# nubot-nudt/MDGAT-matcher

Measured on AMD Instinct MI355X. Metric: keypoint-pairs/sec, higher is better.
Workload: dtype f32 (products as 3 split-f16 MFMAs, fp32 accumulate)

## Files before the change

mdgat_matcher_amd/csrc/layer.hip:

```cpp
#include <utility>
#include <cstdlib>
#include "common.hpp"
#include "layer_image.hpp"
#include "mma_chain.hpp"
namespace {

constexpr int SLOT_CHUNKS = 17;
constexpr int SLOT_BYTES = SLOT_CHUNKS * 1024;
constexpr int SLOT_HALVES = SLOT_BYTES / 2;
constexpr int NSLOT = 5, LOOKAHEAD = 3;
constexpr int WPTS = 16;
constexpr int TROW = 132;
constexpr int TILE_FLOATS = WPTS * TROW;
constexpr int QKROW = 72;
constexpr int VROW = 24;

typedef f16x8 __attribute__((may_alias)) f16x8_a;
typedef f16x4 __attribute__((may_alias)) f16x4_a;
typedef f32x4 __attribute__((may_alias)) f32x4_a;

template <int NW>
__device__ __forceinline__ void stage_dma_slice(const _Float16* g, unsigned lds_addr, int wave, int lane, int i) {
    const int c = min(wave + NW * i, SLOT_CHUNKS - 1);
    const char* src = reinterpret_cast<const char*>(g) + c * 1024;
    asm volatile("s_mov_b32 m0, %0\n\ts_nop 0\n\tglobal_load_lds_dwordx4 %1, %2"
                 :: "s"(lds_addr + c * 1024), "v"(lane * 16), "s"(src) : "memory");
}
template <int NW> constexpr int dma_slices() { return (SLOT_CHUNKS + NW - 1) / NW; }
template <int NW>
__device__ __forceinline__ void stage_dma(const _Float16* g, unsigned lds_addr, int wave, int lane) {
#pragma unroll
    for (int i = 0; i < dma_slices<NW>(); ++i) stage_dma_slice<NW>(g, lds_addr, wave, lane, i);
}
template <typename F, int... U>
__device__ __forceinline__ void for_each_unit(F&& f, std::integer_sequence<int, U...>) { (f(U), ...); }
template <int N, typename F>
__device__ __forceinline__ void for_units(F&& f) { for_each_unit(f, std::make_integer_sequence<int, N>{}); }

template <int YOUNGER>
__device__ __forceinline__ void stage_wait() {
    asm volatile("s_waitcnt vmcnt(%0)" :: "n"(YOUNGER) : "memory");
    __syncthreads();
}
template <int NW>
__device__ __forceinline__ void end_of_pair(int h1, int nstage) {
    if (h1 + 3 < nstage) stage_wait<dma_slices<NW>()>();
    else stage_wait<0>();
}

struct UnitAcc { f32x4 pm, px, qm, qx; };

template <int NK32, bool SWAP, int ROWH, typename Inter>
__device__ __forceinline__ void unit_mma16(const _Float16* buf, int l15, int g, const f16x8* xh, const f16x8* xl,
                                           UnitAcc& acc, Inter&& inter) {
    constexpr int K = NK32 * 32, AHEAD = 2;
    const _Float16* wp = buf + l15 * ROWH + 8 * g;
    const _Float16* wq = wp + 16 * ROWH;
    acc.pm = f32x4{0.f, 0.f, 0.f, 0.f}; acc.px = acc.pm; acc.qm = acc.pm; acc.qx = acc.pm;
    f16x8 ph[NK32], pl[NK32], qh[NK32], ql[NK32];
#pragma unroll
    for (int ks = 0; ks < AHEAD; ++ks) {
        ph[ks] = *reinterpret_cast<const f16x8*>(wp + 32 * ks);
        pl[ks] = *reinterpret_cast<const f16x8*>(wp + K + 32 * ks);
        qh[ks] = *reinterpret_cast<const f16x8*>(wq + 32 * ks);
        ql[ks] = *reinterpret_cast<const f16x8*>(wq + K + 32 * ks);
    }
    auto mm = [&](const f16x8& w, const f16x8& x, const f32x4& c) __attribute__((always_inline)) {
        return SWAP ? __builtin_amdgcn_mfma_f32_16x16x32_f16(w, x, c, 0, 0, 0)
                    : __builtin_amdgcn_mfma_f32_16x16x32_f16(x, w, c, 0, 0, 0);
    };
#pragma unroll
    for (int ks = 0; ks < NK32; ++ks) {
        if (ks + AHEAD < NK32) {
            ph[ks + AHEAD] = *reinterpret_cast<const f16x8*>(wp + 32 * (ks + AHEAD));
            pl[ks + AHEAD] = *reinterpret_cast<const f16x8*>(wp + K + 32 * (ks + AHEAD));
            qh[ks + AHEAD] = *reinterpret_cast<const f16x8*>(wq + 32 * (ks + AHEAD));
            ql[ks + AHEAD] = *reinterpret_cast<const f16x8*>(wq + K + 32 * (ks + AHEAD));
        }
        __builtin_amdgcn_sched_barrier(0);
        acc.px = mm(ph[ks], xl[ks], acc.px); inter(6 * ks); __builtin_amdgcn_sched_barrier(0);
        acc.qx = mm(qh[ks], xl[ks], acc.qx); inter(6 * ks + 1); __builtin_amdgcn_sched_barrier(0);
        acc.pm = mm(ph[ks], xh[ks], acc.pm); inter(6 * ks + 2); __builtin_amdgcn_sched_barrier(0);
        acc.qm = mm(qh[ks], xh[ks], acc.qm); inter(6 * ks + 3); __builtin_amdgcn_sched_barrier(0);
        acc.px = mm(pl[ks], xh[ks], acc.px); inter(6 * ks + 4); __builtin_amdgcn_sched_barrier(0);
        acc.qx = mm(ql[ks], xh[ks], acc.qx); inter(6 * ks + 5); __builtin_amdgcn_sched_barrier(0);
    }
}

template <int NK32, int ROWH, typename Inter>
__device__ __forceinline__ void block_mma16(const _Float16* buf, int l15, int g, const f16x8* xh, const f16x8* xl,
                                            f32x4& m, f32x4& x, Inter&& inter) {
    constexpr int K = NK32 * 32, AHEAD = 3;
    const _Float16* wp = buf + l15 * ROWH + 8 * g;
    m = f32x4{0.f, 0.f, 0.f, 0.f}; x = m;
    f16x8 ph[NK32], pl[NK32];
#pragma unroll
    for (int ks = 0; ks < AHEAD; ++ks) {
        ph[ks] = *reinterpret_cast<const f16x8*>(wp + 32 * ks);
        pl[ks] = *reinterpret_cast<const f16x8*>(wp + K + 32 * ks);
    }
#pragma unroll
    for (int ks = 0; ks < NK32; ++ks) {
        if (ks + AHEAD < NK32) {
            ph[ks + AHEAD] = *reinterpret_cast<const f16x8*>(wp + 32 * (ks + AHEAD));
            pl[ks + AHEAD] = *reinterpret_cast<const f16x8*>(wp + K + 32 * (ks + AHEAD));
        }
        __builtin_amdgcn_sched_barrier(0);
        x = __builtin_amdgcn_mfma_f32_16x16x32_f16(ph[ks], xl[ks], x, 0, 0, 0); inter(3 * ks); __builtin_amdgcn_sched_barrier(0);
        m = __builtin_amdgcn_mfma_f32_16x16x32_f16(ph[ks], xh[ks], m, 0, 0, 0); inter(3 * ks + 1); __builtin_amdgcn_sched_barrier(0);
        x = __builtin_amdgcn_mfma_f32_16x16x32_f16(pl[ks], xh[ks], x, 0, 0, 0); inter(3 * ks + 2); __builtin_amdgcn_sched_barrier(0);
    }
}

template <int DO_MLP, int MODE3, int VW, int NW>
__global__ __launch_bounds__(64 * NW) void layer_kernel(LayerArgs a) {
    constexpr int NWAVE = NW, DMA_SLICES = dma_slices<NW>();
    static_assert(!VW || NW == 8, "the V^T gather buffers are laid out for 128-keypoint workgroups");
    extern __shared__ __attribute__((aligned(16))) _Float16 smem[];
    const int tid = threadIdx.x;
    const int lane = tid & 63;
    const int wave = __builtin_amdgcn_readfirstlane(tid >> 6);
    const int l15 = lane & 15, g = lane >> 4;
    auto bufp = [&](int i) __attribute__((always_inline)) { return smem + (i % NSLOT) * SLOT_HALVES; };
    const unsigned lds0 = (unsigned)(size_t)(__attribute__((address_space(3))) _Float16*)smem;
    auto ldsb = [&](int i) __attribute__((always_inline)) { return lds0 + (unsigned)(i % NSLOT) * SLOT_BYTES; };
    float* bias1 = reinterpret_cast<float*>(smem + NSLOT * SLOT_HALVES);
    float* bias2 = bias1 + 256;
    float* bias3 = bias2 + 128;
    float* tile = bias3 + 384 + wave * TILE_FLOATS;
    _Float16* tile16 = reinterpret_cast<_Float16*>(tile);
    constexpr int NT = 64 * NWAVE, TILE_PTS = WPTS * NWAVE;
    const int wave_pt0 = blockIdx.x * TILE_PTS + wave * WPTS;
    constexpr int NB3 = MODE3 == 1 ? 12 : 4;

    constexpr int NSTAGE = (DO_MLP ? 24 : 0) + NB3;
    auto stage_src = [&](int h) __attribute__((always_inline)) -> const _Float16* {
        if (DO_MLP && h < 16) return a.w1s + (size_t)h * 16 * ROWH256;
        if (DO_MLP && h < 24) return a.w2s + (size_t)(h - 16) * 16 * ROWH256;
        return a.w3s + (size_t)(h - (DO_MLP ? 24 : 0)) * 32 * ROWH128;
    };
    auto copy_ahead = [&](int h, int i) __attribute__((always_inline)) {
        if (h + LOOKAHEAD < NSTAGE) stage_dma_slice<NW>(stage_src(h + LOOKAHEAD), ldsb(h + LOOKAHEAD), wave, lane, i);
    };
    if (DO_MLP) {
#pragma unroll
        for (int i = tid; i < 256; i += NT) bias1[i] = a.b1[i];
#pragma unroll
        for (int i = tid; i < 128; i += NT) bias2[i] = a.b2[i];
    }
#pragma unroll
    for (int i = tid; i < NB3 * 32; i += NT) bias3[i] = a.b3[i];

    const int l31 = lane & 31, hi = lane >> 5;
    auto rows_load = [&](const float* src, f32x4 (&t)[8]) __attribute__((always_inline)) {
#pragma unroll
        for (int i = 0; i < 8; ++i) {
            const int gp = min(wave_pt0 + 2 * i + hi, a.R - 1);
            t[i] = *reinterpret_cast<const f32x4*>(src + (size_t)gp * 128 + l31 * 4);
        }
    };
    auto rows_guard = [&](const f32x4 (&t)[8], unsigned acc) __attribute__((always_inline)) -> unsigned {
#pragma unroll
        for (int i = 0; i < 8; ++i)
#pragma unroll
            for (int c = 0; c < 4; c += 2)
                acc = max(acc, max(__builtin_bit_cast(unsigned, t[i][c]) & 0x7fffffffu, __builtin_bit_cast(unsigned, t[i][c + 1]) & 0x7fffffffu));
        return acc;
    };
    auto guard_report = [&](unsigned acc) __attribute__((always_inline)) {
        if (a.guard && acc >= __builtin_bit_cast(unsigned, MDGAT_F16_GUARD))
            __hip_atomic_store(a.guard, 1u, __ATOMIC_RELAXED, __HIP_MEMORY_SCOPE_SYSTEM);
    };
    auto rows_to_tile = [&](const f32x4 (&t)[8]) __attribute__((always_inline)) {
#pragma unroll
        for (int i = 0; i < 8; ++i) *reinterpret_cast<f32x4_a*>(tile + (2 * i + hi) * TROW + l31 * 4) = t[i];
    };
    auto tile_to_rows = [&](float* dst) __attribute__((always_inline)) {
#pragma unroll
        for (int i = 0; i < 8; ++i) {
            const int p = 2 * i + hi;
            const f32x4 t = *reinterpret_cast<const f32x4_a*>(tile + p * TROW + l31 * 4);
            const int gp = min(wave_pt0 + p, a.R - 1);
            *reinterpret_cast<f32x4*>(dst + (size_t)gp * 128 + l31 * 4) = t;
        }
    };
    auto tile_fragment = [&](int ks, f16x8& h, f16x8& l) __attribute__((always_inline)) {
        float v[8];
        load8(tile + l15 * TROW + 32 * ks + 8 * g, v);
        split8s(v, h, l);
    };

    UnitAcc acc[2];
    float o[8];
    f16x8 xnh[4], xnl[4];

    float pbias[8], pv[8], phf[8];
    float pbias_v[2] = {0.f, 0.f};
    f16x8 sth, stl;
    f32x4 pback[2];
    constexpr int E_STEPS = 16;

    auto combine = [&](const UnitAcc& c, int half) __attribute__((always_inline)) {
#pragma unroll
        for (int r = 0; r < 4; ++r)
            o[4 * half + r] = half == 0 ? fmaf(c.px[r], MDGAT_SPLIT_INV, c.pm[r]) : fmaf(c.qx[r], MDGAT_SPLIT_INV, c.qm[r]);
    };
    auto load_bias8 = [&](const float* b) __attribute__((always_inline)) { load8(b + 8 * g, pbias); };
    auto split_step = [&](int s_, f16x8& h, f16x8& l, bool SCALED = true) __attribute__((always_inline)) {
        typedef unsigned u32x4 __attribute__((ext_vector_type(4)));
        if (s_ == 0) {
#pragma unroll
            for (int j = 0; j < 8; ++j) h[j] = (_Float16)pv[j];
        } else if (s_ == 1) {
            const u32x4 hp = __builtin_bit_cast(u32x4, h);
#pragma unroll
            for (int j = 0; j < 4; ++j) {
                asm("v_fma_mix_f32 %0, %1, 1.0, -%2 op_sel:[0,0,0] op_sel_hi:[0,0,1]" : "=v"(pv[2 * j]) : "v"(pv[2 * j]), "v"(hp[j]));
                asm("v_fma_mix_f32 %0, %1, 1.0, -%2 op_sel:[0,0,1] op_sel_hi:[0,0,1]" : "=v"(pv[2 * j + 1]) : "v"(pv[2 * j + 1]), "v"(hp[j]));
            }
        } else if (s_ == 2) {
            if (SCALED) {
#pragma unroll
                for (int j = 0; j < 8; ++j) pv[j] *= MDGAT_SPLIT_SCALE;
            }
        } else if (s_ == 3) {
#pragma unroll
            for (int j = 0; j < 8; ++j) l[j] = (_Float16)pv[j];
        }
    };

    constexpr int VSH_OFF = 16 * QKROW, VSHROW = 136, VSH_BUF = 8 * VSHROW;
    _Float16* tiles16 = reinterpret_cast<_Float16*>(bias3 + 384);
    auto vsh = [&](int b, int row, int col) __attribute__((always_inline)) {
        return tiles16 + (row >> 3) * (2 * TILE_FLOATS) + VSH_OFF + b * VSH_BUF + (row & 7) * VSHROW + col;
    };
    auto vstore = [&](int qb, int u) __attribute__((always_inline)) {
        const int p = u >> 1, rl = 4 * p + g;
        if ((u & 1) == 0) pback[p] = *reinterpret_cast<const f32x4_a*>(tile16 + VSH_OFF + (qb & 1) * VSH_BUF + rl * VSHROW + l15 * 8);
        else {
            const int P = a.N + a.M;
            const int pt0 = blockIdx.x * (WPTS * NWAVE);
            const int bb = pt0 / P, pp = pt0 - bb * P;
            const int col0 = pp < a.N ? pp : a.Npad + pp - a.N;
            _Float16* base = a.vt16 + (((size_t)bb * 4 + (qb & 3)) * 64 + 8 * wave + rl) * a.PP + col0;
            *reinterpret_cast<f32x4*>(base + l15 * 8) = pback[p];
        }
    };

    auto e3 = [&](int qb, const UnitAcc& c, int u) __attribute__((always_inline)) {
        if (u == 1 || u == 2) { combine(c, u - 1); return; }
        if (MODE3 == 1 && qb < 8) {
            if (u == 0) load_bias8(bias3 + qb * 32);
            else if (u == 3) {
#pragma unroll
                for (int j = 0; j < 8; ++j) pv[j] = o[j] + pbias[j];
            } else if (u == 4) {
                if (qb < 4) {
#pragma unroll
                    for (int j = 0; j < 8; ++j) pv[j] *= MDGAT_LOG2E * 0.17677669529663687f;
                }
            } else if (u <= 9) split_step(u - 5, sth, stl, false);
            else if (u == 10) {
                *reinterpret_cast<f16x8_a*>(tile16 + l15 * QKROW + 8 * g) = sth;
                *reinterpret_cast<f16x8_a*>(tile16 + l15 * QKROW + 32 + 8 * g) = stl;
            } else if (u == 11) {
#pragma unroll
                for (int p = 0; p < 2; ++p)
                    pback[p] = *reinterpret_cast<const f32x4_a*>(tile16 + (8 * p + (lane >> 3)) * QKROW + (lane & 7) * 8);
            } else if (u <= 13) {
                const int p = u - 12;
                _Float16* dst = (qb < 4 ? a.q16 : a.k16) + (size_t)(qb & 3) * 64;
                const int row = 8 * p + (lane >> 3), cc = lane & 7;
                const int gp = min(wave_pt0 + row, a.R - 1);
                *reinterpret_cast<f32x4*>(dst + (size_t)gp * 256 + cc * 8) = pback[p];
            }
        } else if (MODE3 == 1) {
            const int head = qb & 3;
            const int P = a.N + a.M;
            if (VW) {
                if (u == 0) { pbias_v[0] = bias3[qb * 32 + l15]; pbias_v[1] = bias3[qb * 32 + 16 + l15]; }
                else if (u == 3) {
#pragma unroll
                    for (int j = 0; j < 8; ++j) pv[j] = o[j] + pbias_v[j >> 2];
                } else if (u >= 5 && u <= 9) split_step(u - 5, sth, stl, false);
                else if (u == 10) {
                    _Float16* c0 = vsh(qb & 1, l15, 16 * wave + 4 * g);
                    *reinterpret_cast<f16x4_a*>(c0) = f16x4{sth[0], sth[1], sth[2], sth[3]};
                    *reinterpret_cast<f16x4_a*>(c0 + 2 * 2 * TILE_FLOATS) = f16x4{sth[4], sth[5], sth[6], sth[7]};
                    *reinterpret_cast<f16x4_a*>(c0 + 4 * 2 * TILE_FLOATS) = f16x4{stl[0], stl[1], stl[2], stl[3]};
                    *reinterpret_cast<f16x4_a*>(c0 + 6 * 2 * TILE_FLOATS) = f16x4{stl[4], stl[5], stl[6], stl[7]};
                }
            } else if (((a.N | a.M) & 15) == 0) {
                if (wave_pt0 < a.R) {
                    if (u == 0) { pbias_v[0] = bias3[qb * 32 + l15]; pbias_v[1] = bias3[qb * 32 + 16 + l15]; }
                    else if (u == 3) {
#pragma unroll
                        for (int j = 0; j < 8; ++j) pv[j] = o[j] + pbias_v[j >> 2];
                    } else if (u >= 5 && u <= 9) split_step(u - 5, sth, stl, false);
                    else if (u == 10) {
                        *reinterpret_cast<f16x4_a*>(tile16 + l15 * VROW + 4 * g) = f16x4{sth[0], sth[1], sth[2], sth[3]};
                        *reinterpret_cast<f16x4_a*>(tile16 + (16 + l15) * VROW + 4 * g) = f16x4{sth[4], sth[5], sth[6], sth[7]};
                        *reinterpret_cast<f16x4_a*>(tile16 + (32 + l15) * VROW + 4 * g) = f16x4{stl[0], stl[1], stl[2], stl[3]};
                        *reinterpret_cast<f16x4_a*>(tile16 + (48 + l15) * VROW + 4 * g) = f16x4{stl[4], stl[5], stl[6], stl[7]};
                    } else if (u == 11) {
#pragma unroll
                        for (int p = 0; p < 2; ++p)
                            pback[p] = *reinterpret_cast<const f32x4_a*>(tile16 + lane * VROW + p * 8);
                    } else if (u == 12 || u == 13) {
                        const int p = u - 12;
                        const int bb = wave_pt0 / P, pp = wave_pt0 - bb * P;
                        const int col0 = pp < a.N ? pp : a.Npad + pp - a.N;
                        _Float16* base = a.vt16 + ((size_t)bb * 4 + head) * 64 * a.PP + col0;
                        *reinterpret_cast<f32x4*>(base + (size_t)lane * a.PP + p * 8) = pback[p];
                    }
                }
            } else if (u == 11) {
                const bool fast = ((a.N | a.M) & 3) == 0;
                const int p0 = wave_pt0 + 4 * g;
#pragma unroll
                for (int blk = 0; blk < 2; ++blk) {
                    if (p0 >= a.R) continue;
                    const int dim = 16 * blk + l15;
                    const float bias = bias3[qb * 32 + dim];
                    _Float16 h[4], l[4];
#pragma unroll
                    for (int j = 0; j < 4; ++j) mdgat_split_unscaled(o[4 * blk + j] + bias, h[j], l[j]);
                    if (fast) {
                        const int bb = p0 / P, pp = p0 - bb * P;
                        _Float16* row_h = a.vt16 + (((size_t)bb * 4 + head) * 2 * 32 + dim) * a.PP;
                        const int col = pp < a.N ? pp : a.Npad + pp - a.N;
                        *reinterpret_cast<f16x4*>(row_h + col) = f16x4{h[0], h[1], h[2], h[3]};
                        *reinterpret_cast<f16x4*>(row_h + (size_t)32 * a.PP + col) = f16x4{l[0], l[1], l[2], l[3]};
                    } else {
#pragma unroll
                        for (int j = 0; j < 4; ++j) {
                            const int pj = p0 + j;
                            if (pj >= a.R) break;
                            const int bj = pj / P, qj = pj - bj * P;
                            const int col = qj < a.N ? qj : a.Npad + qj - a.N;
                            _Float16* rh = a.vt16 + (((size_t)bj * 4 + head) * 2 * 32 + dim) * a.PP;
                            rh[col] = h[j];
                            rh[(size_t)32 * a.PP + col] = l[j];
                        }
                    }
                }
            }
        } else {
            if (u == 0) load_bias8(bias3 + qb * 32);
            else if (u == 3) {
#pragma unroll
                for (int j = 0; j < 8; ++j) pv[j] = o[j] + pbias[j];
            } else if (u == 4) store8(tile + l15 * TROW + qb * 32 + 8 * g, pv);
        }
    };

    if (DO_MLP) {
        f16x8 ah[8], al[8];
        {
            f32x4 tm[8], tx[8];
            rows_load(a.msg, tm);
            rows_load(a.x, tx);
            for_units<LOOKAHEAD>([&](int h) __attribute__((always_inline)) { stage_dma<NW>(stage_src(h), ldsb(h), wave, lane); });
            rows_to_tile(tm);
            const unsigned gm = rows_guard(tm, 0u);
            for_units<4>([&](int ks) __attribute__((always_inline)) { tile_fragment(ks, ah[4 + ks], al[4 + ks]); });
            rows_to_tile(tx);
            guard_report(rows_guard(tx, gm));
        }
        for_units<4>([&](int ks) __attribute__((always_inline)) { tile_fragment(ks, ah[ks], al[ks]); });
        stage_wait<DMA_SLICES>();

        f16x8 hh[8], hl[8];
        auto e1 = [&](int rb, const UnitAcc& c, int u) __attribute__((always_inline)) {
            if (u == 0) load_bias8(bias1 + rb * 32);
            else if (u <= 2) combine(c, u - 1);
            else if (u == 3) {
#pragma unroll
                for (int j = 0; j < 8; ++j) pv[j] = o[j] + pbias[j];
            } else if (u == 4) {
#pragma unroll
                for (int j = 0; j < 8; ++j) pv[j] = fmaxf(pv[j], 0.f);
            } else if (u <= 9) split_step(u - 5, hh[rb], hl[rb]);
        };
        for_units<8>([&](int rb) __attribute__((always_inline)) {
            auto inter = [&](int h, int base) __attribute__((always_inline)) {
                return [&, h, base](int slot) __attribute__((always_inline)) {
                    if (slot % 4 == 1 && slot / 4 < DMA_SLICES) copy_ahead(h, slot / 4);
                    if (slot % 2 == 0 && rb > 0) e1(rb - 1, acc[(rb - 1) & 1], (base + slot) / 2);
                };
            };
            block_mma16<8, ROWH256>(bufp(2 * rb), l15, g, ah, al, acc[rb & 1].pm, acc[rb & 1].px, inter(2 * rb, 0));
            block_mma16<8, ROWH256>(bufp(2 * rb + 1), l15, g, ah, al, acc[rb & 1].qm, acc[rb & 1].qx, inter(2 * rb + 1, 24));
            end_of_pair<NW>(2 * rb + 1, NSTAGE);
        });

        auto e2 = [&](int ob, const UnitAcc& c, int u) __attribute__((always_inline)) {
            if (u == 0) {
                load_bias8(bias2 + ob * 32);
                load8(tile + l15 * TROW + ob * 32 + 8 * g, phf);
            } else if (u <= 2) combine(c, u - 1);
            else if (u == 3) {
#pragma unroll
                for (int j = 0; j < 8; ++j) pv[j] = o[j] + pbias[j];
            } else if (u == 4) {
#pragma unroll
                for (int j = 0; j < 8; ++j) pv[j] += phf[j];
            } else if (u == 5) store8(tile + l15 * TROW + ob * 32 + 8 * g, pv);
            else if (u <= 10) split_step(u - 6, xnh[ob], xnl[ob]);
        };
        for_units<4>([&](int ob) __attribute__((always_inline)) {
            constexpr int H0 = 16;
            auto inter = [&](int h, int base) __attribute__((always_inline)) {
                return [&, h, base](int slot) __attribute__((always_inline)) {
                    if (slot % 4 == 1 && slot / 4 < DMA_SLICES) copy_ahead(h, slot / 4);
                    if (slot % 2 != 0) return;
                    if (ob == 0) e1(7, acc[1], (base + slot) / 2);
                    else e2(ob - 1, acc[(ob - 1) & 1], (base + slot) / 2);
                };
            };
            block_mma16<8, ROWH256>(bufp(H0 + 2 * ob), l15, g, hh, hl, acc[ob & 1].pm, acc[ob & 1].px, inter(H0 + 2 * ob, 0));
            block_mma16<8, ROWH256>(bufp(H0 + 2 * ob + 1), l15, g, hh, hl, acc[ob & 1].qm, acc[ob & 1].qx, inter(H0 + 2 * ob + 1, 24));
            end_of_pair<NW>(H0 + 2 * ob + 1, NSTAGE);
        });
        for_units<E_STEPS>([&](int u) __attribute__((always_inline)) { e2(3, acc[1], u); });
        tile_to_rows(a.x);
    } else {
        {
            f32x4 tx[8];
            rows_load(a.x, tx);
            for_units<LOOKAHEAD>([&](int h) __attribute__((always_inline)) { stage_dma<NW>(stage_src(h), ldsb(h), wave, lane); });
            rows_to_tile(tx);
            guard_report(rows_guard(tx, 0u));
        }
        for_units<4>([&](int ks) __attribute__((always_inline)) { tile_fragment(ks, xnh[ks], xnl[ks]); });
        stage_wait<DMA_SLICES>();
    }

    for_units<NB3>([&](int q) __attribute__((always_inline)) {
        constexpr int H0 = DO_MLP ? 24 : 0;
        const _Float16* cur = bufp(H0 + q);
        auto inter = [&](int slot) __attribute__((always_inline)) {
            if (slot % 4 == 1 && slot / 4 < DMA_SLICES) copy_ahead(H0 + q, slot / 4);
            if (q > 0) e3(q - 1, acc[(q - 1) & 1], slot);
            if (VW && q >= 10 && slot >= 18 && slot < 22) vstore(q - 2, slot - 18);
        };
        if (MODE3 == 1 && q >= 8) unit_mma16<4, false, ROWH128>(cur, l15, g, xnh, xnl, acc[q & 1], inter);
        else unit_mma16<4, true, ROWH128>(cur, l15, g, xnh, xnl, acc[q & 1], inter);
        if ((q & 1) && q + 1 < NB3) end_of_pair<NW>(H0 + q, NSTAGE);
        else if (VW && q >= 10) __syncthreads();
    });
    if (VW) for_units<4>([&](int u) __attribute__((always_inline)) { vstore(NB3 - 2, u); });
    for_units<E_STEPS>([&](int u) __attribute__((always_inline)) { e3(NB3 - 1, acc[(NB3 - 1) & 1], u); });
    if (VW) {
        __syncthreads();
        for_units<4>([&](int u) __attribute__((always_inline)) { vstore(NB3 - 1, u); });
    }
    if (MODE3 != 1) tile_to_rows(a.mdesc);
}

__global__ __launch_bounds__(256) void split_rows_kernel(const float* w, _Float16* out, int rows, int K, int rowh, int nperm) {
    const size_t total = (size_t)rows * K;
    for (size_t i = (size_t)blockIdx.x * 256 + threadIdx.x; i < total; i += (size_t)gridDim.x * 256) {
        const int r = (int)(i / K), c = (int)(i - (size_t)r * K);
        int src = r;
        if (r < nperm) {
            const int j = r & 15, q = (r >> 4) & 1;
            src = (r & ~31) + 8 * (j >> 2) + 4 * q + (j & 3);
        }
        _Float16 h, l;
        mdgat_split(w[(size_t)src * K + c], h, l);
        out[(size_t)r * rowh + c] = h;
        out[(size_t)r * rowh + K + c] = l;
    }
}

template <int DO_MLP, int MODE3, int VW, int NW>
int launch_layer_t(const LayerArgs& a, hipStream_t s) {
    constexpr int NWAVE = NW;
    const size_t lds = (size_t)NSLOT * SLOT_BYTES + (768 + NWAVE * TILE_FLOATS) * sizeof(float);
    static std::atomic<unsigned long long> optin;
    if (int rc = mdgat_lds_optin(reinterpret_cast<const void*>(layer_kernel<DO_MLP, MODE3, VW, NW>), lds, optin, "layer LDS attribute")) return rc;
    constexpr int TILE_PTS = WPTS * NWAVE;
    hipLaunchKernelGGL((layer_kernel<DO_MLP, MODE3, VW, NW>), dim3((a.R + TILE_PTS - 1) / TILE_PTS), dim3(64 * NWAVE), lds, s, a);
    return mdgat_check_hip(hipGetLastError(), "layer launch");
}

}

int launch_split_rows(const float* w, _Float16* out, int rows, int K, int rowh, int nperm, hipStream_t s) {
    const size_t total = (size_t)rows * K;
    const int blocks = (int)((total + 255) / 256 < 1024 ? (total + 255) / 256 : 1024);
    hipLaunchKernelGGL(split_rows_kernel, dim3(blocks), dim3(256), 0, s, w, out, rows, K, rowh, nperm);
    return mdgat_check_hip(hipGetLastError(), "split_rows launch");
}

static std::atomic<int> g_split_tiles{[] { const char* e = getenv("MDGAT_LAYER_SPLIT_TILES"); return e ? atoi(e) : MDGAT_LAYER_SPLIT_TILES_DEFAULT; }()};
extern "C" int mdgat_set_layer_split_tiles(int tiles) { return g_split_tiles.exchange(tiles < 0 ? MDGAT_LAYER_SPLIT_TILES_DEFAULT : tiles); }

int launch_layer(const LayerLaunch& p, hipStream_t s) {
    if (p.R <= 0) return MDGAT_OK;
    LayerArgs a{};
    a.x = p.x; a.msg = p.msg;
    a.w1s = p.mlp.w1s; a.b1 = p.mlp.b1; a.w2s = p.mlp.w2s; a.b2 = p.mlp.b2; a.w3s = p.proj.w3s; a.b3 = p.proj.b3;
    a.w1f = p.mlp.w1f; a.w2f = p.mlp.w2f; a.w3f = p.proj.w3f;
    a.q16 = p.out.q16; a.k16 = p.out.k16; a.vt16 = p.out.vt16; a.mdesc = p.mdesc;
    a.R = p.R; a.N = p.N; a.M = p.M; a.Npad = p.out.Npad; a.PP = p.out.PP; a.guard = p.guard;
    if ((p.R + 127) / 128 <= g_split_tiles.load(std::memory_order_relaxed)) return launch_layer_split(a, p.do_mlp, p.proj.mode3, s);
    if ((p.R + 127) / 128 <= MDGAT_LAYER_TILE64_TILES) {
        if (p.do_mlp) return p.proj.mode3 != 1 ? launch_layer_t<1, 2, 0, 4>(a, s) : launch_layer_t<1, 1, 0, 4>(a, s);
        return p.proj.mode3 != 1 ? launch_layer_t<0, 2, 0, 4>(a, s) : launch_layer_t<0, 1, 0, 4>(a, s);
    }
    const bool vw = p.proj.mode3 == 1 && ((p.N | p.M) & 127) == 0;
    if (p.do_mlp) return p.proj.mode3 != 1 ? launch_layer_t<1, 2, 0, 8>(a, s) : vw ? launch_layer_t<1, 1, 1, 8>(a, s) : launch_layer_t<1, 1, 0, 8>(a, s);
    return p.proj.mode3 != 1 ? launch_layer_t<0, 2, 0, 8>(a, s) : vw ? launch_layer_t<0, 1, 1, 8>(a, s) : launch_layer_t<0, 1, 0, 8>(a, s);
}
```

Before: 21310.

## Replace per-wave LDS transpose tiles with cross-lane permutes and direct register stores

Removes the per-wave fp32 LDS tile used to transpose rows into MFMA fragments and back. Input rows are loaded in a layout where ds_bpermute and permlane16_swap move data into fragment ownership, and outputs (mdesc, x residual, q/k/v f16) are stored straight from registers. The residual is kept in registers, and the V^T gather buffer is placed in a free weight ring slot. This cuts LDS footprint (a static_assert sizes it so an attention workgroup can share the CU) and LDS round trips, at the cost of more permute instructions, held registers, and narrower global stores.

```diff
diff --git a/mdgat_matcher_amd/csrc/layer.hip b/mdgat_matcher_amd/csrc/layer.hip
--- a/mdgat_matcher_amd/csrc/layer.hip
+++ b/mdgat_matcher_amd/csrc/layer.hip
@@ -10,14 +10,11 @@
 constexpr int SLOT_HALVES = SLOT_BYTES / 2;
 constexpr int NSLOT = 5, LOOKAHEAD = 3;
 constexpr int WPTS = 16;
-constexpr int TROW = 132;
-constexpr int TILE_FLOATS = WPTS * TROW;
-constexpr int QKROW = 72;
-constexpr int VROW = 24;
-
-typedef f16x8 __attribute__((may_alias)) f16x8_a;
+constexpr int LAYER_LDS_BYTES = NSLOT * SLOT_BYTES + 768 * (int)sizeof(float);
+static_assert(LAYER_LDS_BYTES <= 163840 - 67584, "the layer kernel shares its CU's LDS with one attention_stream_kernel workgroup");
 typedef f16x4 __attribute__((may_alias)) f16x4_a;
 typedef f32x4 __attribute__((may_alias)) f32x4_a;
+typedef unsigned u32x4 __attribute__((ext_vector_type(4)));
 
 template <int NW>
 __device__ __forceinline__ void stage_dma_slice(const _Float16* g, unsigned lds_addr, int wave, int lane, int i) {
@@ -115,7 +112,7 @@
 template <int DO_MLP, int MODE3, int VW, int NW>
 __global__ __launch_bounds__(64 * NW) void layer_kernel(LayerArgs a) {
     constexpr int NWAVE = NW, DMA_SLICES = dma_slices<NW>();
-    static_assert(!VW || NW == 8, "the V^T gather buffers are laid out for 128-keypoint workgroups");
+    static_assert(!VW || (NW == 8 && MODE3 == 1), "the V^T gather buffers are laid out for 128-keypoint workgroups");
     extern __shared__ __attribute__((aligned(16))) _Float16 smem[];
     const int tid = threadIdx.x;
     const int lane = tid & 63;
@@ -127,8 +124,6 @@
     float* bias1 = reinterpret_cast<float*>(smem + NSLOT * SLOT_HALVES);
     float* bias2 = bias1 + 256;
     float* bias3 = bias2 + 128;
-    float* tile = bias3 + 384 + wave * TILE_FLOATS;
-    _Float16* tile16 = reinterpret_cast<_Float16*>(tile);
     constexpr int NT = 64 * NWAVE, TILE_PTS = WPTS * NWAVE;
     const int wave_pt0 = blockIdx.x * TILE_PTS + wave * WPTS;
     constexpr int NB3 = MODE3 == 1 ? 12 : 4;
@@ -151,13 +146,28 @@
 #pragma unroll
     for (int i = tid; i < NB3 * 32; i += NT) bias3[i] = a.b3[i];
 
-    const int l31 = lane & 31, hi = lane >> 5;
+    const int gp = min(wave_pt0 + l15, a.R - 1);
     auto rows_load = [&](const float* src, f32x4 (&t)[8]) __attribute__((always_inline)) {
+        const float* row = src + (size_t)min(wave_pt0 + (lane >> 2), a.R - 1) * 128 + 8 * (lane & 3);
+#pragma unroll
+        for (int i = 0; i < 8; ++i) t[i] = *reinterpret_cast<const f32x4*>(row + 32 * (i >> 1) + 4 * (i & 1));
+    };
+    auto rows_own = [&](f32x4 (&t)[8]) __attribute__((always_inline)) {
+        const int from = 4 * (4 * l15 + g);
 #pragma unroll
         for (int i = 0; i < 8; ++i) {
-            const int gp = min(wave_pt0 + 2 * i + hi, a.R - 1);
-            t[i] = *reinterpret_cast<const f32x4*>(src + (size_t)gp * 128 + l31 * 4);
-        }
+            const u32x4 w = __builtin_bit_cast(u32x4, t[i]);
+            u32x4 r;
+#pragma unroll
+            for (int d = 0; d < 4; ++d) r[d] = (unsigned)__builtin_amdgcn_ds_bpermute(from, (int)w[d]);
+            t[i] = __builtin_bit_cast(f32x4, r);
+        }
+    };
+    auto late = [&](int v) __attribute__((always_inline)) { asm volatile("" : "+v"(v)); return v; };
+    auto unit_store = [&](float* dst, int unit, const float (&v)[8]) __attribute__((always_inline)) {
+        float* row = dst + (size_t)late(gp) * 128 + 32 * unit + 8 * g;
+        *reinterpret_cast<f32x4*>(row) = f32x4{v[0], v[1], v[2], v[3]};
+        *reinterpret_cast<f32x4*>(row + 4) = f32x4{v[4], v[5], v[6], v[7]};
     };
     auto rows_guard = [&](const f32x4 (&t)[8], unsigned acc) __attribute__((always_inline)) -> unsigned {
 #pragma unroll
@@ -171,22 +181,8 @@
         if (a.guard && acc >= __builtin_bit_cast(unsigned, MDGAT_F16_GUARD))
             __hip_atomic_store(a.guard, 1u, __ATOMIC_RELAXED, __HIP_MEMORY_SCOPE_SYSTEM);
     };
-    auto rows_to_tile = [&](const f32x4 (&t)[8]) __attribute__((always_inline)) {
-#pragma unroll
-        for (int i = 0; i < 8; ++i) *reinterpret_cast<f32x4_a*>(tile + (2 * i + hi) * TROW + l31 * 4) = t[i];
-    };
-    auto tile_to_rows = [&](float* dst) __attribute__((always_inline)) {
-#pragma unroll
-        for (int i = 0; i < 8; ++i) {
-            const int p = 2 * i + hi;
-            const f32x4 t = *reinterpret_cast<const f32x4_a*>(tile + p * TROW + l31 * 4);
-            const int gp = min(wave_pt0 + p, a.R - 1);
-            *reinterpret_cast<f32x4*>(dst + (size_t)gp * 128 + l31 * 4) = t;
-        }
-    };
-    auto tile_fragment = [&](int ks, f16x8& h, f16x8& l) __attribute__((always_inline)) {
-        float v[8];
-        load8(tile + l15 * TROW + 32 * ks + 8 * g, v);
+    auto rows_fragment = [&](const f32x4 (&t)[8], int ks, f16x8& h, f16x8& l) __attribute__((always_inline)) {
+        const float v[8] = {t[2 * ks][0], t[2 * ks][1], t[2 * ks][2], t[2 * ks][3], t[2 * ks + 1][0], t[2 * ks + 1][1], t[2 * ks + 1][2], t[2 * ks + 1][3]};
         split8s(v, h, l);
     };
 
@@ -194,7 +190,7 @@
     float o[8];
     f16x8 xnh[4], xnl[4];
 
-    float pbias[8], pv[8], phf[8];
+    float pbias[8], pv[8];
     float pbias_v[2] = {0.f, 0.f};
     f16x8 sth, stl;
     f32x4 pback[2];
@@ -229,14 +225,14 @@
         }
     };
 
-    constexpr int VSH_OFF = 16 * QKROW, VSHROW = 136, VSH_BUF = 8 * VSHROW;
-    _Float16* tiles16 = reinterpret_cast<_Float16*>(bias3 + 384);
-    auto vsh = [&](int b, int row, int col) __attribute__((always_inline)) {
-        return tiles16 + (row >> 3) * (2 * TILE_FLOATS) + VSH_OFF + b * VSH_BUF + (row & 7) * VSHROW + col;
+    constexpr int VSHROW = 136;
+    static_assert(64 * VSHROW * 2 <= SLOT_BYTES, "a V^T gather buffer is one ring slot");
+    auto vsh = [&](int qb, int row, int col) __attribute__((always_inline)) {
+        return smem + (((DO_MLP ? 24 : 0) + qb - 1) % NSLOT) * SLOT_HALVES + row * VSHROW + col;
     };
     auto vstore = [&](int qb, int u) __attribute__((always_inline)) {
         const int p = u >> 1, rl = 4 * p + g;
-        if ((u & 1) == 0) pback[p] = *reinterpret_cast<const f32x4_a*>(tile16 + VSH_OFF + (qb & 1) * VSH_BUF + rl * VSHROW + l15 * 8);
+        if ((u & 1) == 0) pback[p] = *reinterpret_cast<const f32x4_a*>(vsh(qb, 8 * wave + rl, l15 * 8));
         else {
             const int P = a.N + a.M;
             const int pt0 = blockIdx.x * (WPTS * NWAVE);
@@ -246,7 +242,12 @@
             *reinterpret_cast<f32x4*>(base + l15 * 8) = pback[p];
         }
     };
-
+    auto lanes_gather = [&](int src, const f16x8& v) __attribute__((always_inline)) {
+        u32x4 w = __builtin_bit_cast(u32x4, v);
+#pragma unroll
+        for (int d = 0; d < 4; ++d) w[d] = (unsigned)__builtin_amdgcn_ds_bpermute(src, (int)w[d]);
+        return __builtin_bit_cast(f16x8, w);
+    };
     auto e3 = [&](int qb, const UnitAcc& c, int u) __attribute__((always_inline)) {
         if (u == 1 || u == 2) { combine(c, u - 1); return; }
         if (MODE3 == 1 && qb < 8) {
@@ -261,18 +262,12 @@
                 }
             } else if (u <= 9) split_step(u - 5, sth, stl, false);
             else if (u == 10) {
-                *reinterpret_cast<f16x8_a*>(tile16 + l15 * QKROW + 8 * g) = sth;
-                *reinterpret_cast<f16x8_a*>(tile16 + l15 * QKROW + 32 + 8 * g) = stl;
-            } else if (u == 11) {
-#pragma unroll
-                for (int p = 0; p < 2; ++p)
-                    pback[p] = *reinterpret_cast<const f32x4_a*>(tile16 + (8 * p + (lane >> 3)) * QKROW + (lane & 7) * 8);
-            } else if (u <= 13) {
-                const int p = u - 12;
-                _Float16* dst = (qb < 4 ? a.q16 : a.k16) + (size_t)(qb & 3) * 64;
-                const int row = 8 * p + (lane >> 3), cc = lane & 7;
-                const int gp = min(wave_pt0 + row, a.R - 1);
-                *reinterpret_cast<f32x4*>(dst + (size_t)gp * 256 + cc * 8) = pback[p];
+                const int t = late(lane), src = 4 * ((t >> 2) + 16 * (t & 3));
+                sth = lanes_gather(src, sth); stl = lanes_gather(src, stl);
+            } else if (u == 12 || u == 13) {
+                const int t = late(lane), row = min(wave_pt0 + (t >> 2), a.R - 1);
+                _Float16* dst = (qb < 4 ? a.q16 : a.k16) + (size_t)row * 256 + (qb & 3) * 64 + 8 * (t & 3);
+                *reinterpret_cast<f16x8*>(dst + 32 * (u - 12)) = u == 12 ? sth : stl;
             }
         } else if (MODE3 == 1) {
             const int head = qb & 3;
@@ -284,11 +279,11 @@
                     for (int j = 0; j < 8; ++j) pv[j] = o[j] + pbias_v[j >> 2];
                 } else if (u >= 5 && u <= 9) split_step(u - 5, sth, stl, false);
                 else if (u == 10) {
-                    _Float16* c0 = vsh(qb & 1, l15, 16 * wave + 4 * g);
+                    _Float16* c0 = vsh(qb, l15, 16 * wave + 4 * g);
                     *reinterpret_cast<f16x4_a*>(c0) = f16x4{sth[0], sth[1], sth[2], sth[3]};
-                    *reinterpret_cast<f16x4_a*>(c0 + 2 * 2 * TILE_FLOATS) = f16x4{sth[4], sth[5], sth[6], sth[7]};
-                    *reinterpret_cast<f16x4_a*>(c0 + 4 * 2 * TILE_FLOATS) = f16x4{stl[0], stl[1], stl[2], stl[3]};
-                    *reinterpret_cast<f16x4_a*>(c0 + 6 * 2 * TILE_FLOATS) = f16x4{stl[4], stl[5], stl[6], stl[7]};
+                    *reinterpret_cast<f16x4_a*>(c0 + 16 * VSHROW) = f16x4{sth[4], sth[5], sth[6], sth[7]};
+                    *reinterpret_cast<f16x4_a*>(c0 + 32 * VSHROW) = f16x4{stl[0], stl[1], stl[2], stl[3]};
+                    *reinterpret_cast<f16x4_a*>(c0 + 48 * VSHROW) = f16x4{stl[4], stl[5], stl[6], stl[7]};
                 }
             } else if (((a.N | a.M) & 15) == 0) {
                 if (wave_pt0 < a.R) {
@@ -298,20 +293,23 @@
                         for (int j = 0; j < 8; ++j) pv[j] = o[j] + pbias_v[j >> 2];
                     } else if (u >= 5 && u <= 9) split_step(u - 5, sth, stl, false);
                     else if (u == 10) {
-                        *reinterpret_cast<f16x4_a*>(tile16 + l15 * VROW + 4 * g) = f16x4{sth[0], sth[1], sth[2], sth[3]};
-                        *reinterpret_cast<f16x4_a*>(tile16 + (16 + l15) * VROW + 4 * g) = f16x4{sth[4], sth[5], sth[6], sth[7]};
-                        *reinterpret_cast<f16x4_a*>(tile16 + (32 + l15) * VROW + 4 * g) = f16x4{stl[0], stl[1], stl[2], stl[3]};
-                        *reinterpret_cast<f16x4_a*>(tile16 + (48 + l15) * VROW + 4 * g) = f16x4{stl[4], stl[5], stl[6], stl[7]};
+                        u32x4 sh = __builtin_bit_cast(u32x4, sth), sl = __builtin_bit_cast(u32x4, stl);
+#pragma unroll
+                        for (int d = 0; d < 4; ++d) {
+                            u32x4& s2 = d < 2 ? sh : sl;
+                            const auto r = __builtin_amdgcn_permlane16_swap(s2[d & 1], s2[2 + (d & 1)], false, false);
+                            s2[d & 1] = r[0]; s2[2 + (d & 1)] = r[1];
+                        }
+                        sth = __builtin_bit_cast(f16x8, sh); stl = __builtin_bit_cast(f16x8, sl);
                     } else if (u == 11) {
-#pragma unroll
-                        for (int p = 0; p < 2; ++p)
-                            pback[p] = *reinterpret_cast<const f32x4_a*>(tile16 + lane * VROW + p * 8);
+                        const int t = late(lane), src = 4 * (32 * (t & 1) + (t >> 1));
+                        sth = lanes_gather(src, sth); stl = lanes_gather(src, stl);
                     } else if (u == 12 || u == 13) {
-                        const int p = u - 12;
                         const int bb = wave_pt0 / P, pp = wave_pt0 - bb * P;
                         const int col0 = pp < a.N ? pp : a.Npad + pp - a.N;
                         _Float16* base = a.vt16 + ((size_t)bb * 4 + head) * 64 * a.PP + col0;
-                        *reinterpret_cast<f32x4*>(base + (size_t)lane * a.PP + p * 8) = pback[p];
+                        const int t = late(lane);
+                        *reinterpret_cast<f16x8*>(base + (size_t)(32 * (u - 12) + (t >> 1)) * a.PP + 8 * (t & 1)) = u == 12 ? sth : stl;
                     }
                 }
             } else if (u == 11) {
@@ -350,31 +348,33 @@
             else if (u == 3) {
 #pragma unroll
                 for (int j = 0; j < 8; ++j) pv[j] = o[j] + pbias[j];
-            } else if (u == 4) store8(tile + l15 * TROW + qb * 32 + 8 * g, pv);
+            } else if (u == 4) unit_store(a.mdesc, qb, pv);
         }
     };
 
     if (DO_MLP) {
         f16x8 ah[8], al[8];
+        f32x4 xr[8];
         {
-            f32x4 tm[8], tx[8];
+            f32x4 tm[8];
             rows_load(a.msg, tm);
-            rows_load(a.x, tx);
+            rows_load(a.x, xr);
             for_units<LOOKAHEAD>([&](int h) __attribute__((always_inline)) { stage_dma<NW>(stage_src(h), ldsb(h), wave, lane); });
-            rows_to_tile(tm);
+            rows_own(tm);
             const unsigned gm = rows_guard(tm, 0u);
-            for_units<4>([&](int ks) __attribute__((always_inline)) { tile_fragment(ks, ah[4 + ks], al[4 + ks]); });
-            rows_to_tile(tx);
-            guard_report(rows_guard(tx, gm));
-        }
-        for_units<4>([&](int ks) __attribute__((always_inline)) { tile_fragment(ks, ah[ks], al[ks]); });
+            for_units<4>([&](int ks) __attribute__((always_inline)) { rows_fragment(tm, ks, ah[4 + ks], al[4 + ks]); });
+            rows_own(xr);
+            guard_report(rows_guard(xr, gm));
+        }
+        for_units<4>([&](int ks) __attribute__((always_inline)) { rows_fragment(xr, ks, ah[ks], al[ks]); });
         stage_wait<DMA_SLICES>();
 
         f16x8 hh[8], hl[8];
         auto e1 = [&](int rb, const UnitAcc& c, int u) __attribute__((always_inline)) {
-            if (u == 0) load_bias8(bias1 + rb * 32);
-            else if (u <= 2) combine(c, u - 1);
-            else if (u == 3) {
+            if (u == 1 || u == 2) {
+                combine(c, u - 1);
+                if (u == 2) load_bias8(bias1 + rb * 32);
+            } else if (u == 3) {
 #pragma unroll
                 for (int j = 0; j < 8; ++j) pv[j] = o[j] + pbias[j];
             } else if (u == 4) {
@@ -395,17 +395,15 @@
         });
 
         auto e2 = [&](int ob, const UnitAcc& c, int u) __attribute__((always_inline)) {
-            if (u == 0) {
-                load_bias8(bias2 + ob * 32);
-                load8(tile + l15 * TROW + ob * 32 + 8 * g, phf);
-            } else if (u <= 2) combine(c, u - 1);
+            if (u == 0) load_bias8(bias2 + ob * 32);
+            else if (u <= 2) combine(c, u - 1);
             else if (u == 3) {
 #pragma unroll
                 for (int j = 0; j < 8; ++j) pv[j] = o[j] + pbias[j];
             } else if (u == 4) {
 #pragma unroll
-                for (int j = 0; j < 8; ++j) pv[j] += phf[j];
-            } else if (u == 5) store8(tile + l15 * TROW + ob * 32 + 8 * g, pv);
+                for (int j = 0; j < 8; ++j) pv[j] += xr[2 * ob + (j >> 2)][j & 3];
+            } else if (u == 5) unit_store(a.x, ob, pv);
             else if (u <= 10) split_step(u - 6, xnh[ob], xnl[ob]);
         };
         for_units<4>([&](int ob) __attribute__((always_inline)) {
@@ -423,16 +421,15 @@
             end_of_pair<NW>(H0 + 2 * ob + 1, NSTAGE);
         });
         for_units<E_STEPS>([&](int u) __attribute__((always_inline)) { e2(3, acc[1], u); });
-        tile_to_rows(a.x);
     } else {
         {
             f32x4 tx[8];
             rows_load(a.x, tx);
             for_units<LOOKAHEAD>([&](int h) __attribute__((always_inline)) { stage_dma<NW>(stage_src(h), ldsb(h), wave, lane); });
-            rows_to_tile(tx);
+            rows_own(tx);
             guard_report(rows_guard(tx, 0u));
-        }
-        for_units<4>([&](int ks) __attribute__((always_inline)) { tile_fragment(ks, xnh[ks], xnl[ks]); });
+            for_units<4>([&](int ks) __attribute__((always_inline)) { rows_fragment(tx, ks, xnh[ks], xnl[ks]); });
+        }
         stage_wait<DMA_SLICES>();
     }
 
@@ -455,7 +452,6 @@
         __syncthreads();
         for_units<4>([&](int u) __attribute__((always_inline)) { vstore(NB3 - 1, u); });
     }
-    if (MODE3 != 1) tile_to_rows(a.mdesc);
 }
 
 __global__ __launch_bounds__(256) void split_rows_kernel(const float* w, _Float16* out, int rows, int K, int rowh, int nperm) {
@@ -477,7 +473,7 @@
 template <int DO_MLP, int MODE3, int VW, int NW>
 int launch_layer_t(const LayerArgs& a, hipStream_t s) {
     constexpr int NWAVE = NW;
-    const size_t lds = (size_t)NSLOT * SLOT_BYTES + (768 + NWAVE * TILE_FLOATS) * sizeof(float);
+    constexpr size_t lds = LAYER_LDS_BYTES;
     static std::atomic<unsigned long long> optin;
     if (int rc = mdgat_lds_optin(reinterpret_cast<const void*>(layer_kernel<DO_MLP, MODE3, VW, NW>), lds, optin, "layer LDS attribute")) return rc;
     constexpr int TILE_PTS = WPTS * NWAVE;
```

Result: no change. 21290 (-0.1%).
